# LauraBaracaldo/LauraBaracaldo-Spatial-Meta-Kriging-for-Distributed-Inference-for-Binary-Response

Measured on AMD Instinct MI355X. Metric: MCMC iters/sec (all subsets, whole node) + end-to-end wall-clock, n=500k K=250, higher is better.
Workload: dtype f64

## Files before the change

laurabaracaldo-spatial-meta-kriging-for-distributed-inference-for-binary-response_amd/csrc/mk_gemm.hpp:

```cpp
#pragma once
#include "mk_common.hpp"

namespace mk {

typedef double d4 __attribute__((ext_vector_type(4)));
typedef double d2 __attribute__((ext_vector_type(2)));

constexpr int GB_K = 16;
__host__ __device__ constexpr int gb_stride(int len) {
  return len == 256 ? 272 : (len == 128 ? 144 : (len == 64 ? 80 : 48));
}
__host__ __device__ constexpr int gb_img(int len) { return GB_K * gb_stride(len); }
__host__ __device__ constexpr int gb_lds_bytes(int tm, int tn) { return 2 * (gb_img(tm) + gb_img(tn)) * 8; }
static_assert(gb_lds_bytes(128, 128) == MK_GD_LDS_BYTES, "mk_common.hpp LDS size");
static_assert(128 * GB_K <= gb_img(128) && 64 * GB_K <= gb_img(64) && 32 * GB_K <= gb_img(32),
              "k-contiguous images fit their slots");

template <int BM, int BN>
struct AccT {
  d4 v[BM][BN];
};
typedef AccT<4, 4> Acc;

template <int BM, int BN>
__device__ inline void acc_zero(AccT<BM, BN>& a) {
#pragma unroll
  for (int i = 0; i < BM; ++i)
#pragma unroll
    for (int j = 0; j < BN; ++j) a.v[i][j] = (d4){0.0, 0.0, 0.0, 0.0};
}

__device__ inline int ku_swz(int m) { return (m >> 1) & 7; }

template <bool MU, int LEN>
__host__ __device__ constexpr int dma_count() { return MU ? 4 * (LEN > 128 ? LEN / 128 : 1) : (LEN + 31) / 32; }

template <bool MU, int LEN>
__device__ inline void dma_chunk(const double* __restrict__ X, long s, int k0, double* img) {
  const int w = threadIdx.x >> 6, lane = threadIdx.x & 63;
  if (MU) {
    static_assert(!MU || LEN <= 128 || LEN % 128 == 0, "m-contiguous rows of 128-double pieces");
#pragma unroll
    for (int j = 0; j < 4; ++j) {
      const int r = w + 4 * j;
#pragma unroll
      for (int pc = 0; pc < (LEN > 128 ? LEN / 128 : 1); ++pc)
        if (LEN >= 128 || lane < LEN / 2)
          __builtin_amdgcn_global_load_lds((const void*)(X + (long)(k0 + r) * s + 128 * pc + 2 * lane),
                                           (void*)(img + r * gb_stride(LEN) + 128 * pc), 16, 0, 0);
    }
  } else {
#pragma unroll
    for (int j = 0; j < (LEN + 31) / 32; ++j) {
// ... 116 lines not shown
  const int lane = threadIdx.x & 63, w = threadIdx.x >> 6;
  const int li = lane & 15, lk = lane >> 4;
#pragma unroll
  for (int ks = 0; ks < GB_K / 4; ++ks) {
    const int k = ks * 4 + lk;
    double ya[BM], xb[8];
#pragma unroll
    for (int b = 0; b < BM; ++b) {
      const double av = frag<true, TM>(As, w * (TM / 4) + b * 16 + li, k);
      ya[b] = NEG ? -av : av;
    }
#pragma unroll
    for (int b = 0; b < 8; ++b) xb[b] = frag<true, 128>(Bs, b * 16 + li, k);
#pragma unroll
    for (int bm = 0; bm < BM; ++bm)
#pragma unroll
      for (int bn = 0; bn < 8; ++bn)
        acc.v[bm][bn] = __builtin_amdgcn_mfma_f64_16x16x4f64(xb[bn], ya[bm], acc.v[bm][bn], 0, 0, 0);
  }
}

template <int TM, bool NEG>
__device__ inline void gemm_tile_rw(const double* __restrict__ A, long sA, const double* __restrict__ B, long sB, int K,
                                    AccRW<TM>& acc, double* lds) {
  constexpr int STAGE = gb_img(TM) + gb_img(128);
  const int nch = K / GB_K;
  auto issue = [&](int c) {
    double* st = lds + (c & 1) * STAGE;
    dma_chunk<true, TM>(A, sA, GB_K * c, st);
    dma_chunk<true, 128>(B, sB, GB_K * c, st + gb_img(TM));
  };
  issue(0);
  asm volatile("s_waitcnt vmcnt(0)" ::: "memory");
  __syncthreads();
  for (int c = 0; c < nch; ++c) {
    const double* st = lds + (c & 1) * STAGE;
    if (c + 1 < nch) issue(c + 1);
    mma_chunk_rw<TM, NEG>(st, st + gb_img(TM), acc);
    asm volatile("s_waitcnt vmcnt(0)" ::: "memory");
    __syncthreads();
  }
}

template <int TM>
__device__ inline void acc_load_rw(AccRW<TM>& acc, const double* C, long ldc) {
#pragma unroll
  for (int bm = 0; bm < TM / 64; ++bm)
#pragma unroll
    for (int bn = 0; bn < 8; ++bn)
#pragma unroll
      for (int r = 0; r < 4; ++r) acc.v[bm][bn][r] = C[rw_row<TM>(bm) + (long)rw_col(bn, r) * ldc];
}

template <bool A_MU, bool B_NU, bool NEG = false, bool REV = false, bool SAME = false, int SKIP = SKIP_NONE,
          bool MASK = false>
__device__ inline void gemm_128(const double* __restrict__ A, long sA, const double* __restrict__ B, long sB, int K,
                                int kvalid_total, Acc& acc, double* lds, int diag_tile = 0) {
  gemm_tile<128, 128, A_MU, B_NU, NEG, REV, SAME, SKIP, MASK>(A, sA, B, sB, K, kvalid_total, acc, lds, diag_tile);
}

template <int TM = 128>
__device__ inline int acc_row(int bm) {
  const int lane = threadIdx.x & 63, wm = (threadIdx.x >> 6) & 1;
  return wm * (TM / 2) + bm * 16 + (lane & 15);
}
template <int TN = 128>
__device__ inline int acc_col(int bn, int r) {
  const int lane = threadIdx.x & 63, wn = threadIdx.x >> 7;
  return wn * (TN / 2) + bn * 16 + (lane >> 4) + 4 * r;
}

template <int BM, int BN>
__device__ inline void acc_load(AccT<BM, BN>& acc, const double* C, long ldc) {
#pragma unroll
  for (int bm = 0; bm < BM; ++bm)
#pragma unroll
    for (int bn = 0; bn < BN; ++bn)
#pragma unroll
      for (int r = 0; r < 4; ++r) acc.v[bm][bn][r] = C[acc_row<BM * 32>(bm) + (long)acc_col<BN * 32>(bn, r) * ldc];
}

template <int BM, int BN>
__device__ inline void store_tile(double* C, long ldc, const AccT<BM, BN>& acc, double* Ct = nullptr) {
#pragma unroll
  for (int bm = 0; bm < BM; ++bm)
#pragma unroll
    for (int bn = 0; bn < BN; ++bn)
#pragma unroll
      for (int r = 0; r < 4; ++r) {
        const int m = acc_row<BM * 32>(bm), n = acc_col<BN * 32>(bn, r);
        C[m + (long)n * ldc] = acc.v[bm][bn][r];
        if (Ct) Ct[n + (long)m * ldc] = acc.v[bm][bn][r];
      }
}

constexpr int SYRK_SLOTS = 9;
__host__ __device__ constexpr int syrk_rb(int w, int s) { return s <= w ? w : 7 - w; }
__host__ __device__ constexpr int syrk_cb(int w, int s) { return s <= w ? s : s - w - 1; }
constexpr bool syrk_cover_exact() {
  int cnt[8][8] = {};
  for (int w = 0; w < 4; ++w)
    for (int s = 0; s < SYRK_SLOTS; ++s) {
      const int rb = syrk_rb(w, s), cb = syrk_cb(w, s);
      if (rb < 0 || rb > 7 || cb < 0 || cb > rb) return false;
      ++cnt[rb][cb];
    }
// ... 217 lines not shown
```

laurabaracaldo-spatial-meta-kriging-for-distributed-inference-for-binary-response_amd/csrc/mk_kernels.hpp:

```cpp
#pragma once
#include "mk_types.hpp"
#include "mk_corr.hpp"

namespace mk {
inline int xcd_grid_h(int S, int T) { return 8 * ((S + 7) / 8) * T; }
template <int MODEL>
__global__ void k_cov_candidate(Model md, MatSet ms, int h0, int hc, int which, int iter, const int* slist, const int* scount);
typedef void (*CovCandidateKernel)(Model, MatSet, int, int, int, int, const int*, const int*);
inline CovCandidateKernel cov_candidate_kernel(int model) {
  return model == MK_COV_EXPONENTIAL ? k_cov_candidate<MK_COV_EXPONENTIAL> : k_cov_candidate<MK_COV_MATERN>;
}
template <int TM, int TN = TM>
__global__ void k_chol_update(MatSet ms, int S, int h0, int hc, int k, int ia, int ib, int j0, int j1,
                              const int* slist, const int* scount, int syrk);
template <int TM>
__global__ void k_chol_trsm(MatSet ms, int S, int h0, int hc, int k, int ia, int ib, const int* slist,
                            const int* scount);
int pv_grid(int max_entries, int nt, int ntt);
template <int TM>
__global__ void k_chol_update_trsm(MatSet ms, int S, int h0, int hc, int k, int ia, int ib, int j0, int extra,
                                   const int* slist, const int* scount, int syrk);
__global__ void k_chol_diag(MatSet ms, const int* n_s, int h0, int hc, int k, double* ld_part, double* quad_c, int* info,
                            const int* slist, const int* scount, int cj0, int cj1, int syrk);
__global__ void k_inv_copydiag(MatSet ms, const int* list, const int* count);
template <int TM>
__global__ void k_inv_level(MatSet ms, const int* list, const int* count, int sz, int phase, int deal, int map);
__global__ void k_lauum(MatSet ms, const int* n_s, const int* list, const int* count);
__global__ void k_qblocks(MatSet ms, const int* n_s, const int* list, const int* count);
__global__ void k_take_border(Model md, MatSet ms, const int* list, const int* count, const double* zc);
__global__ void k_cand_border(Model md, MatSet ms, int h0, int hc);
__global__ void k_pred_draw_runs(Model md, const double* kz, const double* kA, int k_lo, const int* plist,
                                 const int* pcount, const int* run_start, int j_end);
__global__ void k_run_start(const int* plist, const int* pcount, int* run_start, int j);
__global__ void k_border_step(Model md, MatSet ms, int k);
__global__ void k_nu_border(Model md, MatSet ms);
__global__ void k_border_quad(Model md);
__global__ void k_trmv_Z(Model md, MatSet ms);
template <int MODEL>
__global__ void k_pred_PT(Model md, const int* list, const int* count);
__global__ void k_pred_PT_matern(Model md, const int* list, const int* count);
__global__ void k_matern_table(Model md, int h0, int hc, int which, int iter, const int* slist, const int* scount);
__global__ void k_matern_table_list(Model md, const int* list, const int* count);
typedef void (*PredPTKernel)(Model, const int*, const int*);
inline PredPTKernel pred_PT_kernel(int model) {
  return model == MK_COV_EXPONENTIAL ? k_pred_PT<MK_COV_EXPONENTIAL> : k_pred_PT<MK_COV_MATERN>;
}
template <bool GEN>
__global__ void k_pred_var(Model md, MatSet ms, const int* list, const int* count);
__global__ void k_pred_var_reduce(Model md, int nt, const int* list, const int* count);
__global__ void k_beta(Model md, int iter);
__global__ void k_Aphase(Model md, int iter);
__global__ void k_theta_mh(Model md, MatSet ms, int h0, int hc, int which, int iter);
__global__ void k_dirty_list(Model md, int force, int* list_inv, int* count_inv, int* list_pred, int* count_pred);
template <int Q>
__global__ void k_sweep(Model md, MatSet ms, int iter, const int* adm, int* fb);
template <int Q>
__global__ void k_sweep_mg(Model md, MatSet ms, int iter, double* part, int* cnt, int* xcc, int* err, int* adm, int spins_max);
template <int Q, int KR, int P, int HH, int LN>
__global__ void k_sweep_site(Model md, MatSet ms, int iter);
inline size_t sweep_site_lds_bytes(int ns_max, int q, int lean = 0) { return (size_t)ns_max * q * (lean ? 4 : 3) * 8 + (size_t)ns_max * 4; }
inline const void* sweep_site_kernel(int q, int kr, int lean = 1) {
  if (q == 1) {
    if (kr == 1)
      return lean == 1 ? (const void*)k_sweep_site<1, 4, 2, 0, 1> : (const void*)k_sweep_site<1, 4, 2, 0, 2>;
    return lean == 1 ? (const void*)k_sweep_site<1, 8, 2, 0, 1> : (const void*)k_sweep_site<1, 8, 2, 0, 2>;
  }
  switch (q) {
    case 2: return kr == 1 ? (const void*)k_sweep_site<2, 4, 1, 0, 0> : (const void*)k_sweep_site<2, 8, 1, 0, 0>;
    case 3: return kr == 1 ? (const void*)k_sweep_site<3, 4, 1, 0, 0> : nullptr;
    default: return nullptr;
  }
}
template <int Q>
__global__ void k_sweep_step(Model md, MatSet ms, int iter, int B, double* part);
// ... 72 lines not shown
```

laurabaracaldo-spatial-meta-kriging-for-distributed-inference-for-binary-response_amd/csrc/mk_linalg.hip:

```cpp
#include "mk_gemm.hpp"
#include "mk_types.hpp"
#include "mk_corr.hpp"

namespace mk {

__device__ inline void candidate_theta(const Model& md, int s, int h, int which, int iter, double* phi, double* nu) {
  const Key key = subset_key(md, s);
  const double* th = md.theta + (long)s * md.n_theta;
  const int idx_phi = md.ntri + h, idx_nu = md.ntri + md.q + h;
  double tphi = th[idx_phi];
  double tnu = (md.cov_model == MK_COV_MATERN) ? th[idx_nu] : 0.0;
  if (which == 0 || which == 1) {
    const int j_mh = (which == 0) ? md.o_phi + h : md.o_nu + h;
    const double z = proposal_normal(key, (uint32_t)j_mh, (uint32_t)iter);
    const double step = exp(md.tune[(long)s * md.n_mh_max + j_mh]) * z;
    if (which == 0) tphi += step; else tnu += step;
  }
  *phi = logit_inv(tphi, md.phi_a[h], md.phi_b[h]);
  *nu = (md.cov_model == MK_COV_MATERN) ? logit_inv(tnu, md.nu_a[h], md.nu_b[h]) : 0.0;
}

struct CandGen {
  const double* cx;
  const double* cy;
// ... 220 lines not shown
  const int sr = st % SUBR, sc = st / SUBR;
  const int i = ia + t;
  if (i == k && sc * TN >= (sr + 1) * TM) return;
  const int sh = s * ms.q + h;
  double* M = mat_slot(ms, sh, 1 - ms.cur[sh]);
  const long ld = ms.ld;
  double* C = M + i * MK_NB + sr * TM + (long)(k * MK_NB + sc * TN) * ld;
  const long jo = (long)j0 * MK_NB * ld;
  if (TM == 128 && TN == 128 && i == k && syrk) {
    AccSyrk a;
    acc_load_syrk(a, C, ld);
    gemm_syrk_128(M + i * MK_NB + jo, ld, (j1 - j0) * MK_NB, a, lds);
    store_tile_syrk(C, ld, a);
    return;
  }
  AccT<TM / 32, TN / 32> acc;
  acc_load(acc, C, ld);
  gemm_tile<TM, TN, true, true, true>(M + i * MK_NB + sr * TM + jo, ld, M + k * MK_NB + sc * TN + jo, ld,
                                      (j1 - j0) * MK_NB, (j1 - j0) * MK_NB, acc, lds);
  store_tile(C, ld, acc);
}
template __global__ void k_chol_update<128, 128>(MatSet, int, int, int, int, int, int, int, int, const int*, const int*, int);
template __global__ void k_chol_update<64, 64>(MatSet, int, int, int, int, int, int, int, int, const int*, const int*, int);
template __global__ void k_chol_update<32, 32>(MatSet, int, int, int, int, int, int, int, int, const int*, const int*, int);

template <int TM>
__global__ __launch_bounds__(256, 2) void k_chol_trsm(MatSet ms, int S, int h0, int hc, int k, int ia, int ib,
                                                     const int* slist, const int* scount) {
  extern __shared__ __attribute__((aligned(16))) double lds[];
  constexpr int SUB = MK_NB / TM;
  const int ntk = ib - ia;
  int e, t, s, h;
  if (!xcd_map(active_pairs(slist, scount, S, hc), ntk * SUB, &e, &t) || !pick_pair(slist, scount, e, h0, hc, &s, &h))
    return;
  const int sr = t % SUB;
  t /= SUB;
  const int i = ia + t;
  const int sh = s * ms.q + h;
  const int slot = 1 - ms.cur[sh];
  double* M = mat_slot(ms, sh, slot);
  const double* W = winv_slot(ms, sh, slot, k);
  const long ld = ms.ld;
  double* C = M + i * MK_NB + sr * TM + (long)k * MK_NB * ld;
  AccT<TM / 32, 4> acc;
  acc_zero(acc);
  gemm_tile<TM, 128, true, true, false, false, false, SKIP_TRI_B>(C, ld, W, MK_NB, MK_NB, MK_NB, acc, lds);
  store_tile(C, ld, acc);
}
template __global__ void k_chol_trsm<128>(MatSet, int, int, int, int, int, int, const int*, const int*);
template __global__ void k_chol_trsm<64>(MatSet, int, int, int, int, int, int, const int*, const int*);
template __global__ void k_chol_trsm<32>(MatSet, int, int, int, int, int, int, const int*, const int*);

template <int TM>
__global__ __launch_bounds__(256, 2) void k_chol_update_trsm(MatSet ms, int S, int h0, int hc, int k, int ia, int ib,
                                                            int j0, int extra, const int* slist, const int* scount,
                                                            int syrk) {
  extern __shared__ __attribute__((aligned(16))) double lds[];
  constexpr int SUB = MK_NB / TM, BM = TM / 64;
  const int ntk = ib - ia;
  int e, t, s, h;
  const int E = active_pairs(slist, scount, S, hc);
  if (!((extra && syrk) ? xcd_map_tail(E, ntk * SUB + extra, &e, &t) : xcd_map(E, ntk * SUB + extra, &e, &t)) ||
      !pick_pair(slist, scount, e, h0, hc, &s, &h))
    return;
  const int sh = s * ms.q + h;
  const int slot = 1 - ms.cur[sh];
  double* M = mat_slot(ms, sh, slot);
  const long ld = ms.ld;
  if (t == ntk * SUB) {
    double* C = M + ia * MK_NB + (long)ia * MK_NB * ld;
    if (syrk) {
      AccSyrk a;
      acc_load_syrk(a, C, ld);
      gemm_syrk_128(M + ia * MK_NB, ld, k * MK_NB, a, lds);
      store_tile_syrk(C, ld, a);
      return;
    }
    Acc acc;
    acc_load(acc, C, ld);
    gemm_tile<128, 128, true, true, true>(M + ia * MK_NB, ld, M + ia * MK_NB, ld, k * MK_NB, k * MK_NB, acc, lds);
    store_tile(C, ld, acc);
    return;
  }
  const int i = ia + t / SUB, r0 = i * MK_NB + (t % SUB) * TM;
  double* C = M + r0 + (long)k * MK_NB * ld;
  AccRW<TM> c;
  acc_load_rw<TM>(c, C, ld);
  const long jo = (long)j0 * MK_NB * ld;
  gemm_tile_rw<TM, true>(M + r0 + jo, ld, M + k * MK_NB + jo, ld, (k - j0) * MK_NB, c, lds);
  double* Co = C;
  long ldo = ld;
  asm volatile("" : "+s"(Co), "+s"(ldo));
  const double* Wt = winv_slot(ms, sh, slot, k);
  asm volatile("" : "+s"(Wt));
  constexpr int IMG = gb_img(32);
  auto issue = [&](int P, double* buf) {
#pragma nounroll
    for (int ch = 0; ch < 2 * P + 2; ++ch) dma_chunk<true, 32>(Wt + 32 * P, MK_NB, GB_K * ch, buf + ch * IMG);
  };
  double* bufA = lds;
  double* bufB = lds + 8 * IMG;
  issue(3, bufA);
  asm volatile("s_waitcnt vmcnt(0)" ::: "memory");
  __syncthreads();
  const int lane = threadIdx.x & 63, li = lane & 15, lk = lane >> 4;
#pragma unroll
  for (int idx = 0; idx < 4; ++idx) {
    const int P = idx == 0 ? 3 : (idx == 1 ? 0 : (idx == 2 ? 2 : 1));
    const double* buf = (idx & 1) ? bufB : bufA;
    if (idx < 3) {
      const int Pn = idx == 0 ? 0 : (idx == 1 ? 2 : 1);
      issue(Pn, (idx & 1) ? bufA : bufB);
    }
    AccT<BM, 2> o;
    acc_zero(o);
#pragma unroll
    for (int ch = 0; ch < 8; ++ch) {
      if (ch >= 2 * P + 2) break;
#pragma unroll
      for (int ks = 0; ks < GB_K / 4; ++ks) {
        const int kk = ks * 4 + lk;
        double xb[2];
#pragma unroll
        for (int b = 0; b < 2; ++b) xb[b] = frag<true, 32>(buf + ch * IMG, b * 16 + li, kk);
#pragma unroll
        for (int bm = 0; bm < BM; ++bm)
#pragma unroll
          for (int b = 0; b < 2; ++b) {
            if (ch > 2 * P + b) continue;
            o.v[bm][b] = __builtin_amdgcn_mfma_f64_16x16x4f64(xb[b], c.v[bm][ch][ks], o.v[bm][b], 0, 0, 0);
          }
      }
    }
#pragma unroll
    for (int bm = 0; bm < BM; ++bm)
#pragma unroll
      for (int b = 0; b < 2; ++b)
#pragma unroll
        for (int r = 0; r < 4; ++r) Co[rw_row<TM>(bm) + (long)rw_col(2 * P + b, r) * ldo] = o.v[bm][b][r];
    asm volatile("s_waitcnt vmcnt(0)" ::: "memory");
    __syncthreads();
  }
}
template __global__ void k_chol_update_trsm<128>(MatSet, int, int, int, int, int, int, int, int, const int*, const int*, int);
template __global__ void k_chol_update_trsm<64>(MatSet, int, int, int, int, int, int, int, int, const int*, const int*, int);

#define TLD MK_TLD
#define SLD 17
#ifdef MK_DIAG_TIMING
__device__ long long* mk_diag_ts;
#define MK_TSTAMP(i) do { if (threadIdx.x == 0) mk_diag_ts[blockIdx.x * 128 + (i)] = clock64(); } while (0)
#define MK_TSTAMPW(i, t) do { if (threadIdx.x == (t)) mk_diag_ts[blockIdx.x * 128 + (i)] = clock64(); } while (0)
#else
#define MK_TSTAMP(i) do { } while (0)
#define MK_TSTAMPW(i, t) do { } while (0)
#endif

__device__ inline double rlane(double v, int lane) {
  const long long b = __double_as_longlong(v);
  const int lo = __builtin_amdgcn_readlane((int)(b & 0xffffffffll), lane);
  const int hi = __builtin_amdgcn_readlane((int)(b >> 32), lane);
  return __longlong_as_double(((long long)hi << 32) | (unsigned)lo);
}

template <class FA, class FB>
__device__ inline d4 mfma16(d4 acc, int K, FA fa, FB fb) {
  const int l = threadIdx.x & 63;
  for (int k0 = 0; k0 < K; k0 += 16) {
    double a[4], b[4];
#pragma unroll
    for (int u = 0; u < 4; ++u) {
      a[u] = fa(l & 15, k0 + 4 * u + (l >> 4));
      b[u] = fb(k0 + 4 * u + (l >> 4), l & 15);
    }
#pragma unroll
    for (int u = 0; u < 4; ++u) acc = __builtin_amdgcn_mfma_f64_16x16x4f64(a[u], b[u], acc, 0, 0, 0);
  }
  return acc;
}

template <int N>
__device__ inline double bcast16_t(double v) { return __builtin_amdgcn_update_dpp(v, v, 0x150 + N, 0xf, 0xf, false); }
__device__ __forceinline__ double bcast16(double v, int n) {
  switch (n) {
    case 0: return bcast16_t<0>(v);   case 1: return bcast16_t<1>(v);   case 2: return bcast16_t<2>(v);
    case 3: return bcast16_t<3>(v);   case 4: return bcast16_t<4>(v);   case 5: return bcast16_t<5>(v);
    case 6: return bcast16_t<6>(v);   case 7: return bcast16_t<7>(v);   case 8: return bcast16_t<8>(v);
    case 9: return bcast16_t<9>(v);   case 10: return bcast16_t<10>(v); case 11: return bcast16_t<11>(v);
    case 12: return bcast16_t<12>(v); case 13: return bcast16_t<13>(v); case 14: return bcast16_t<14>(v);
    default: return bcast16_t<15>(v);
  }
}

__device__ inline void rsqrt_sqrt(double a, double* d, double* inv) {
  double y = __builtin_amdgcn_rsq(a);
  double e = fma(-a * y, y, 1.0);
  y = fma(0.5 * y, e, y);
  e = fma(-a * y, y, 1.0);
// ... 949 lines not shown
```

laurabaracaldo-spatial-meta-kriging-for-distributed-inference-for-binary-response_amd/csrc/mk_schedule.hip:

```cpp
#include <hip/hip_runtime.h>
#include <algorithm>
#include <cmath>
#include <vector>
#include "mk_gemm.hpp"
#include "mk_session.hpp"

using namespace mk;

void mk::drain_timers(mk_session* s) {
  std::vector<std::pair<float, float>> upd;
  for (auto& t : s->prof.pending) {
    hipEventSynchronize(t.b);
    float ms = 0.f;
    hipEventElapsedTime(&ms, t.a, t.b);
    if (t.cnt >= 0) t.flops *= (double)s->prof.inv_cnt[t.cnt];
    s->prof.stats[t.which].launches += 1;
    s->prof.stats[t.which].ms += ms;
    s->prof.stats[t.which].flops += t.flops;
    if (t.which == KS_CHOL_UPDATE || t.which == KS_CHOL_UPDATE_SUB) {
      float t0 = 0.f;
      hipEventElapsedTime(&t0, s->prof.pending.front().a, t.a);
      upd.push_back({t0, t0 + ms});
      s->prof.stats[KS_UPDATE_BUSY].launches += 1;
      s->prof.stats[KS_UPDATE_BUSY].flops += t.flops;
// ... 40 lines not shown
  return true;
}

int mk::launch_quantiles(unsigned grid, hipStream_t st, const double* data, long subset_stride, long row_stride,
                         int n_rows, int n_cols, const double* probs, int n_probs, double* out) {
  HIPCHK(hipFuncSetAttribute((const void*)k_quantiles, hipFuncAttributeMaxDynamicSharedMemorySize, MK_QUANT_MAX * 8));
  if (n_rows < 1 || n_rows > MK_QUANT_MAX)
    return set_err(MK_E_ARG, "quantile summaries take 1 .. " + std::to_string(MK_QUANT_MAX) + " kept samples");
  size_t n2 = 1;
  while (n2 < (size_t)n_rows) n2 <<= 1;
  MK_LAUNCH(k_quantiles, dim3(grid), dim3(256), n2 * 8, st, data, subset_stride, row_stride, n_rows, n_cols,
                     probs, n_probs, out);
  HIPCHK(hipGetLastError());
  return 0;
}

int mk::launch_quantiles_prob(unsigned grid, hipStream_t st, const double* data, long subset_stride, long row_stride,
                              int n_rows, int n_cols, const double* probs, int n_probs, double* out, const ProbSrc& ps) {
  HIPCHK(hipFuncSetAttribute((const void*)k_quantiles_prob, hipFuncAttributeMaxDynamicSharedMemorySize, MK_QUANT_MAX * 8));
  if (n_rows < 1 || n_rows > MK_QUANT_MAX)
    return set_err(MK_E_ARG, "quantile summaries take 1 .. " + std::to_string(MK_QUANT_MAX) + " kept samples");
  size_t n2 = 1;
  while (n2 < (size_t)n_rows) n2 <<= 1;
  MK_LAUNCH(k_quantiles_prob, dim3(grid), dim3(256), n2 * 8, st, data, subset_stride, row_stride, n_rows, n_cols,
                     probs, n_probs, out, ps);
  HIPCHK(hipGetLastError());
  return 0;
}

static int tile_size(long wg128) {
  static const int force = env_int("MK_TILE", 0);
  if (force == 32 || force == 64 || force == 128) return force;
  return wg128 >= 256 ? 128 : 64;
}

void mk::launch_candidates(const Model& md, const MatSet& ms, hipStream_t st, int n_entries, int h0, int hc, int which,
                           int iter, const int* slist, const int* scount) {
  if (md.cov_model == MK_COV_MATERN && md.chtab)
    MK_LAUNCH(k_matern_table, dim3(n_entries), dim3(256), 0, st, md, h0, hc, which, iter, slist, scount);
  const int ntiles = ms.nt * (ms.nt + 1) / 2;
  MK_LAUNCH(cov_candidate_kernel(md.cov_model), dim3(xcd_grid_h(n_entries, ntiles)),
                     dim3(256), 0, st, md, ms, h0, hc, which, iter, slist, scount);
}


static int diag_syrk() {
  static const int on = env_int("MK_DIAG_SYRK", 1);
  return on != 0;
}

static int inv_deal() {
  static const int on = env_int("MK_INV_DEAL", 1);
  return on != 0;
}

static int inv_map() {
  static const int on = env_int("MK_INV_MAP", 1);
  return on != 0;
}
static int inv_grid(int map, int max_entries, int nt, int sz, int sub) {
  if (map) return inv_map_grid(max_entries, nt, sz, sub);
  return xcd_grid_h(max_entries, (nt + 2 * sz - 1) / (2 * sz) * sz * sz * sub);
}
extern "C" int mk_inv_map_jobs(int32_t map, int32_t count, int32_t max_entries, int32_t nt, int32_t sz, int32_t phase,
                               int32_t sub, int32_t* out, int32_t cap) {
  const int grid = inv_grid(map, max_entries, nt, sz, sub);
  for (int b = 0; out && b < grid && b < cap; ++b) {
    int e, p, i, j, st;
    const bool job = map ? inv_map_job(count, nt, sz, phase, sub, b, &e, &p, &i, &j, &st)
                         : inv_xcd_job(count, nt, sz, phase, sub, b, &e, &p, &i, &j, &st);
    int32_t* o = out + 5 * (long)b;
    o[0] = job ? e : -1, o[1] = job ? p : -1, o[2] = job ? i : -1, o[3] = job ? j : -1, o[4] = job ? st : -1;
  }
  return grid;
}

static void chol_update(mk_session* s, Group& g, hipStream_t st, int h0, int hc, int k, int ia, int ib, int j0, int j1,
                        const int* slist, const int* scount, double flops) {
  const int E = g.S * hc, nti = ib - ia;
  if (nti <= 0) return;
  const int tm = tile_size((long)E * nti);
  if (tm == 32) {
    timed(s, st, KS_CHOL_UPDATE_SUB, flops, [&] {
      MK_LAUNCH(k_chol_update<32>, dim3(xcd_grid_h(E, nti * 16)), dim3(256), LDS_32, st, g.ms, g.S, h0, hc, k, ia,
                         ib, j0, j1, slist, scount, diag_syrk());
    });
  } else if (tm == 64) {
    timed(s, st, KS_CHOL_UPDATE_SUB, flops, [&] {
      MK_LAUNCH(k_chol_update<64>, dim3(xcd_grid_h(E, nti * 4)), dim3(256), LDS_64, st, g.ms, g.S, h0, hc, k, ia,
                         ib, j0, j1, slist, scount, diag_syrk());
    });
  } else {
    timed(s, st, KS_CHOL_UPDATE, flops, [&] {
      MK_LAUNCH(k_chol_update<128>, dim3(xcd_grid_h(E, nti)), dim3(256), LDS_128, st, g.ms, g.S, h0, hc, k, ia,
                         ib, j0, j1, slist, scount, diag_syrk());
    });
  }
}
static void chol_trsm(mk_session* s, Group& g, hipStream_t st, int h0, int hc, int k, int ia, int ib, const int* slist,
                      const int* scount, double flops) {
  const int E = g.S * hc, nti = ib - ia;
  if (nti <= 0) return;
  const int tm = tile_size((long)E * nti);
  timed(s, st, KS_CHOL_TRSM, flops, [&] {
    if (tm == 32)
      MK_LAUNCH(k_chol_trsm<32>, dim3(xcd_grid_h(E, nti * 4)), dim3(256), LDS_32x128, st, g.ms, g.S, h0, hc, k,
                         ia, ib, slist, scount);
    else if (tm == 64)
      MK_LAUNCH(k_chol_trsm<64>, dim3(xcd_grid_h(E, nti * 2)), dim3(256), LDS_64x128, st, g.ms, g.S, h0, hc, k,
                         ia, ib, slist, scount);
    else
      MK_LAUNCH(k_chol_trsm<128>, dim3(xcd_grid_h(E, nti)), dim3(256), LDS_128, st, g.ms, g.S, h0, hc, k, ia, ib,
                         slist, scount);
  });
}
static void chol_update_trsm(mk_session* s, Group& g, hipStream_t st, int h0, int hc, int k, int j0, int extra,
                             const int* slist, const int* scount, double flops) {
  const int E = g.S * hc, nt = s->nt, nti = nt - (k + 1);
  const int tm = tile_size((long)E * (nti + extra));
  timed(s, st, tm == 128 ? KS_CHOL_UPDATE : KS_CHOL_UPDATE_SUB, flops, [&] {
    if (tm == 128)
      MK_LAUNCH(k_chol_update_trsm<128>, dim3(xcd_grid_h(E, nti + extra)), dim3(256), LDS_128, st, g.ms, g.S, h0, hc,
                k, k + 1, nt, j0, extra, slist, scount, diag_syrk());
    else
      MK_LAUNCH(k_chol_update_trsm<64>, dim3(xcd_grid_h(E, 2 * nti + extra)), dim3(256), LDS_128, st, g.ms, g.S, h0,
                hc, k, k + 1, nt, j0, extra, slist, scount, diag_syrk());
  });
}
static void chol_diag(mk_session* s, Group& g, hipStream_t st, int h0, int hc, int k, const int* slist,
                      const int* scount, int cj0 = 0, int cj1 = 0, double flops = 0.0) {
  timed(s, st, KS_CHOL_DIAG, flops, [&] {
    MK_LAUNCH(k_chol_diag, dim3(g.S * hc), dim3(256), (size_t)MK_DIAG_LDS_BYTES, st, g.ms, g.md.n_s, h0, hc, k,
                       g.md.ld_part, g.md.quad_c, g.md.info, slist, scount, cj0, cj1, diag_syrk());
  });
}

static double panel_flops(mk_session* s, Group& g, int hc, int k, int ia, int ib, bool trsm, int j0 = 0, int j1 = -1) {
  if (j1 < 0) j1 = k;
  double fl = 0.0;
  for (int i = g.s0; i < g.s0 + g.S; ++i) {
    const double nv = (double)s->n_part[i] + 1.0;
    const double cols = std::fmin((double)MK_NB, std::fmax(0.0, nv - (double)k * MK_NB));
    const double depth = std::fmax(0.0, std::fmin((double)j1 * MK_NB, nv) - (double)j0 * MK_NB);
    const bool diag = ia <= k && k < ib;
    const double lo = (double)(diag ? k + 1 : ia) * MK_NB;
    const double rows = std::fmax(0.0, std::fmin(nv, (double)ib * MK_NB) - lo);
    if (trsm)
      fl += rows * cols * cols;
    else
      fl += 2.0 * rows * cols * depth + (diag ? cols * (cols + 1.0) * depth : 0.0);
  }
  return fl * hc;
}

static double inv_level_flops(int n, int nt, int sz, int phase) {
  double fl = 0.0;
  for (int T0 = 0; T0 < nt; T0 += 2 * sz) {
    const double t0 = (double)T0 * MK_NB, b0 = (double)(T0 + sz) * MK_NB, b1 = (double)(T0 + 2 * sz) * MK_NB;
    const double bt = std::fmax(0.0, std::fmin((double)n, b0) - t0), bb = std::fmax(0.0, std::fmin((double)n, b1) - b0);
    fl += phase == 0 ? bb * bt * bt : bb * bb * bt;
  }
  return fl;
}

void mk::launch_cholesky(mk_session* s, Group& g, int h0, int hc, const int* slist, const int* scount,
                         hipStream_t crit, hipEvent_t* evP, int k_lo, int k_hi) {
  const int nt = s->nt;
  if (k_hi < 0) k_hi = nt;
  hipStream_t A = crit ? crit : g.stream;
  static const int fused = env_int("MK_CHOL_FUSED", 1);
  if ((slist || !g.bulk) && fused) {
    for (int k = k_lo; k < k_hi; ++k) {
      const int j0 = k >= 2 ? k - 1 : 0;
      chol_diag(s, g, A, h0, hc, k, slist, scount, j0, k, k > 0 ? panel_flops(s, g, hc, k, k, k + 1, false, j0, k) : 0.0);
      if (k == 0 && nt > 1)
        chol_trsm(s, g, A, h0, hc, 0, 1, nt, slist, scount, panel_flops(s, g, hc, 0, 1, nt, true));
      else if (k > 0 && k < nt - 1)
        chol_update_trsm(s, g, A, h0, hc, k, 0, 1, slist, scount,
                         panel_flops(s, g, hc, k, k + 1, nt, false) + panel_flops(s, g, hc, k, k + 1, nt, true) +
// ... 370 lines not shown
```

laurabaracaldo-spatial-meta-kriging-for-distributed-inference-for-binary-response_amd/csrc/mk_types.hpp:

```cpp
#pragma once
#include "../../include/mk.h"
#include "mk_common.hpp"

#define MK_QMAX 4
#define MK_CD_SPLIT 8
#define MK_QUANT_MAX 16384

namespace mk {

struct Model {
  int S, q, p, n_pad, Np, nt, ntri, n_theta, cov_model;
  int link;
  int o_A, o_phi, o_nu, o_w, n_mh_max;
  int n_batch, batch_length, n_samples, kept0, n_kept;
  int n_test, n_test_pad, ntt;
  int subset_base;
  int S_all;
  int t_off;
  uint64_t seed;
  double accept_rate;
  double phi_a[MK_QMAX], phi_b[MK_QMAX], nu_a[MK_QMAX], nu_b[MK_QMAX];
  double iw_df, iw_S[MK_QMAX * MK_QMAX];
  const int* n_s;
  const double* coords;
// ... 77 lines not shown
  int p, link;
};

struct MapThr {
  double u[MK_MAP_MAXT];
  int J;
};

#define MK_CRIT_ACC 6
struct Crit {
  double* acc;
  double* part;
  double* sbeta;
  int nb;
  int n_cap;
};

__device__ inline long mat_elems(const MatSet& m) { return (long)m.ld * m.ld; }
__device__ inline double* mat_slot(const MatSet& m, int sh, int slot) {
  return m.L + ((long)sh * 2 + slot) * mat_elems(m);
}
__device__ inline double* winv_slot(const MatSet& m, int sh, int slot, int k) {
  return m.Winv + (((long)sh * 2 + slot) * m.nt + k) * (MK_NB * MK_NB);
}
__device__ inline Key subset_key(const Model& md, int s) { return make_key(md.seed, (uint32_t)(md.subset_base + s)); }

__host__ __device__ inline bool xcd_map_at(int b, int S, int T, int* s, int* t) {
  const int W = S * T, C = (W + 7) >> 3;
  const int x = b & 7, j = b >> 3;
  if (j >= C) return false;
  const int w = x * C + j;
  if (w >= W) return false;
  *s = w / T;
  *t = w % T;
  return true;
}
__device__ inline bool xcd_map(int S, int T, int* s, int* t) { return xcd_map_at(blockIdx.x, S, T, s, t); }
__device__ inline bool xcd_map_tail(int S, int T, int* s, int* t) {
  const int x = blockIdx.x & 7, j = blockIdx.x >> 3;
  const int Wr = S * (T - 1), Cr = (Wr + 7) >> 3, Cs = (S + 7) >> 3;
  if (j < Cr) {
    const int w = x * Cr + j;
    if (w >= Wr) return false;
    *s = w / (T - 1);
    *t = w % (T - 1);
    return true;
  }
  const int e = x * Cs + (j - Cr);
  if (j - Cr >= Cs || e >= S) return false;
  *s = e;
  *t = T - 1;
  return true;
}
__host__ inline int xcd_grid(int S, int T) { return 8 * ((S + 7) / 8) * T; }

struct InvShape {
  int sz, phase, sub, F, rl;
  __host__ __device__ int n(int k) const { return sub * (phase == 0 ? F * sz + rl : sz * (F + (rl >= k ? 1 : 0))); }
  __host__ __device__ int items() const { return sub * sz * (F * sz + rl); }
  __host__ __device__ int work() const {
    const int full = sz * (sz + 1) / 2;
    return sub * (phase == 0 ? (F * sz + rl) * full : sz * (F * full + rl * (rl + 1) / 2));
  }
};
__host__ __device__ inline InvShape inv_shape(int nt, int sz, int phase, int sub) {
  InvShape h;
  h.sz = sz;
  h.phase = phase;
  h.sub = sub;
  h.F = nt / (2 * sz);
  const int rem = nt - 2 * sz * h.F;
  h.rl = rem > sz ? rem - sz : 0;
  return h;
}
struct InvPos { int e, k, m; };
__host__ __device__ inline InvPos inv_map_cut(const InvShape& h, int S, int x) {
  InvPos q;
  q.e = (x * S) >> 3;
  const int tl = ((x * S) & 7) * h.work();
  int A = 0;
  for (int k = h.sz; k >= 1; --k) {
    const int nk = h.n(k), num = tl - 8 * A - 4 * k;
    if (nk > 0 && num <= 8 * k * (nk - 1)) {
      q.k = k;
      q.m = num <= 0 ? 0 : (num + 8 * k - 1) / (8 * k);
      return q;
    }
    A += nk * k;
  }
  q.e += 1;
  q.k = h.sz;
  q.m = 0;
  return q;
}
__host__ __device__ inline int inv_before(const InvShape& h, const InvPos& q, int k) {
  return k > q.k ? h.n(k) : (k == q.k ? q.m : 0);
}
__host__ __device__ inline bool inv_map_job(int S, int nt, int sz, int phase, int SUB, int b, int* e, int* p, int* i,
                                            int* j, int* st) {
  if (S <= 0) return false;
  const InvShape h = inv_shape(nt, sz, phase, SUB);
  const int x = b & 7;
  int q = b >> 3;
  const InvPos a = inv_map_cut(h, S, x), z = inv_map_cut(h, S, x + 1);
  for (int k = sz; k >= 1; --k) {
    const int nk = h.n(k), ba = inv_before(h, a, k);
// ... 47 lines not shown
```

Baseline: 12960.

## Skip padded rows in last Cholesky update-trsm tile for ragged subsets

For the 128-row update+trsm kernel, this computes how many 16-row blocks of the last row tile are real data for each subset (from n_s) and runs a column-split GEMM over only those blocks. Results are then reshuffled through LDS into the row-wise accumulator layout and passed to a shared solve epilogue that skips the dead row blocks. A new tail job map schedules the last two tiles separately. The intent is to stop spending MFMA work on padding rows in the ragged final tile, at the cost of an extra LDS transpose, more template instantiations and more register pressure.

```diff
diff --git a/laurabaracaldo-spatial-meta-kriging-for-distributed-inference-for-binary-response_amd/csrc/mk_gemm.hpp b/laurabaracaldo-spatial-meta-kriging-for-distributed-inference-for-binary-response_amd/csrc/mk_gemm.hpp
--- a/laurabaracaldo-spatial-meta-kriging-for-distributed-inference-for-binary-response_amd/csrc/mk_gemm.hpp
+++ b/laurabaracaldo-spatial-meta-kriging-for-distributed-inference-for-binary-response_amd/csrc/mk_gemm.hpp
@@ -1,4 +1,5 @@
 #pragma once
+#include <type_traits>
 #include "mk_common.hpp"
 
 namespace mk {
@@ -221,6 +222,99 @@
       for (int r = 0; r < 4; ++r) acc.v[bm][bn][r] = C[rw_row<TM>(bm) + (long)rw_col(bn, r) * ldc];
 }
 
+template <int V>
+using AccCS = AccT<V, 2>;
+constexpr int CS_VMAX = 6;
+
+template <int V, bool NEG>
+__device__ inline void mma_chunk_cs(const double* As, const double* Bs, AccCS<V>& acc, int w) {
+  const int lane = threadIdx.x & 63;
+  const int li = lane & 15, lk = lane >> 4;
+#pragma unroll
+  for (int ks = 0; ks < GB_K / 4; ++ks) {
+    const int k = ks * 4 + lk;
+    double ya[V], xb[2];
+#pragma unroll
+    for (int b = 0; b < V; ++b) {
+      const double av = frag<true, 128>(As, b * 16 + li, k);
+      ya[b] = NEG ? -av : av;
+    }
+#pragma unroll
+    for (int j = 0; j < 2; ++j) xb[j] = frag<true, 128>(Bs, (2 * w + j) * 16 + li, k);
+#pragma unroll
+    for (int bm = 0; bm < V; ++bm)
+#pragma unroll
+      for (int j = 0; j < 2; ++j)
+        acc.v[bm][j] = __builtin_amdgcn_mfma_f64_16x16x4f64(xb[j], ya[bm], acc.v[bm][j], 0, 0, 0);
+  }
+}
+
+template <int V, bool NEG>
+__device__ inline void gemm_tile_cs(const double* __restrict__ A, long sA, const double* __restrict__ B, long sB, int K,
+                                    AccCS<V>& acc, double* lds, int w) {
+  constexpr int STAGE = 2 * gb_img(128);
+  const int nch = K / GB_K;
+  auto issue = [&](int c) {
+    double* st = lds + (c & 1) * STAGE;
+    dma_chunk<true, 128>(A, sA, GB_K * c, st);
+    dma_chunk<true, 128>(B, sB, GB_K * c, st + gb_img(128));
+  };
+  issue(0);
+  asm volatile("s_waitcnt vmcnt(0)" ::: "memory");
+  __syncthreads();
+  for (int c = 0; c < nch; ++c) {
+    const double* st = lds + (c & 1) * STAGE;
+    if (c + 1 < nch) issue(c + 1);
+    mma_chunk_cs<V, NEG>(st, st + gb_img(128), acc, w);
+    asm volatile("s_waitcnt vmcnt(0)" ::: "memory");
+    __syncthreads();
+  }
+}
+
+template <int V>
+__device__ inline void acc_load_cs(AccCS<V>& acc, const double* C, long ldc, int w) {
+  const int li = threadIdx.x & 15, lk = (threadIdx.x & 63) >> 4;
+#pragma unroll
+  for (int bm = 0; bm < V; ++bm)
+#pragma unroll
+    for (int j = 0; j < 2; ++j)
+#pragma unroll
+      for (int r = 0; r < 4; ++r) acc.v[bm][j][r] = C[16 * bm + li + (long)(16 * (2 * w + j) + lk + 4 * r) * ldc];
+}
+
+template <int V>
+__device__ inline void cs_to_rw(const AccCS<V>& a, AccRW<128>& c, double* lds, int w) {
+  static_assert(V >= 1 && V <= 7 && 4 * V * 2048 <= gb_lds_bytes(128, 128), "a round fits the stages' LDS");
+  d2* img = (d2*)lds;
+  const int lane = threadIdx.x & 63;
+#pragma unroll
+  for (int j = 0; j < 2; ++j) {
+#pragma unroll
+    for (int bm = 0; bm < V; ++bm) {
+      d2* p = img + ((bm * 4 + w) * 64 + lane) * 2;
+      p[0] = (d2){a.v[bm][j][0], a.v[bm][j][1]};
+      p[1] = (d2){a.v[bm][j][2], a.v[bm][j][3]};
+    }
+    __syncthreads();
+#pragma unroll
+    for (int bm = 0; bm < 2; ++bm) {
+      const int rb = 2 * w + bm;
+      if (rb < V) {
+#pragma unroll
+        for (int ws = 0; ws < 4; ++ws) {
+          const d2* p = img + ((rb * 4 + ws) * 64 + lane) * 2;
+          const d2 lo = p[0], hi = p[1];
+          c.v[bm][2 * ws + j] = (d4){lo[0], lo[1], hi[0], hi[1]};
+        }
+      } else {
+#pragma unroll
+        for (int ws = 0; ws < 4; ++ws) c.v[bm][2 * ws + j] = (d4){0.0, 0.0, 0.0, 0.0};
+      }
+    }
+    __syncthreads();
+  }
+}
+
 template <bool A_MU, bool B_NU, bool NEG = false, bool REV = false, bool SAME = false, int SKIP = SKIP_NONE,
           bool MASK = false>
 __device__ inline void gemm_128(const double* __restrict__ A, long sA, const double* __restrict__ B, long sB, int K,
diff --git a/laurabaracaldo-spatial-meta-kriging-for-distributed-inference-for-binary-response_amd/csrc/mk_kernels.hpp b/laurabaracaldo-spatial-meta-kriging-for-distributed-inference-for-binary-response_amd/csrc/mk_kernels.hpp
--- a/laurabaracaldo-spatial-meta-kriging-for-distributed-inference-for-binary-response_amd/csrc/mk_kernels.hpp
+++ b/laurabaracaldo-spatial-meta-kriging-for-distributed-inference-for-binary-response_amd/csrc/mk_kernels.hpp
@@ -19,7 +19,7 @@
 int pv_grid(int max_entries, int nt, int ntt);
 template <int TM>
 __global__ void k_chol_update_trsm(MatSet ms, int S, int h0, int hc, int k, int ia, int ib, int j0, int extra,
-                                   const int* slist, const int* scount, int syrk);
+                                   const int* slist, const int* scount, int syrk, const int* n_s, int ragged);
 __global__ void k_chol_diag(MatSet ms, const int* n_s, int h0, int hc, int k, double* ld_part, double* quad_c, int* info,
                             const int* slist, const int* scount, int cj0, int cj1, int syrk);
 __global__ void k_inv_copydiag(MatSet ms, const int* list, const int* count);
diff --git a/laurabaracaldo-spatial-meta-kriging-for-distributed-inference-for-binary-response_amd/csrc/mk_linalg.hip b/laurabaracaldo-spatial-meta-kriging-for-distributed-inference-for-binary-response_amd/csrc/mk_linalg.hip
--- a/laurabaracaldo-spatial-meta-kriging-for-distributed-inference-for-binary-response_amd/csrc/mk_linalg.hip
+++ b/laurabaracaldo-spatial-meta-kriging-for-distributed-inference-for-binary-response_amd/csrc/mk_linalg.hip
@@ -296,17 +296,81 @@
 template __global__ void k_chol_trsm<32>(MatSet, int, int, int, int, int, int, const int*, const int*);
 
 template <int TM>
+__device__ inline void solve_epilogue_rw(const AccRW<TM>& c, int nbm, double* C, long ld, const double* Wt, double* lds) {
+  constexpr int BM = TM / 64;
+  double* Co = C;
+  long ldo = ld;
+  asm volatile("" : "+s"(Co), "+s"(ldo));
+  asm volatile("" : "+s"(Wt));
+  constexpr int IMG = gb_img(32);
+  auto issue = [&](int P, double* buf) {
+#pragma nounroll
+    for (int ch = 0; ch < 2 * P + 2; ++ch) dma_chunk<true, 32>(Wt + 32 * P, MK_NB, GB_K * ch, buf + ch * IMG);
+  };
+  double* bufA = lds;
+  double* bufB = lds + 8 * IMG;
+  issue(3, bufA);
+  asm volatile("s_waitcnt vmcnt(0)" ::: "memory");
+  __syncthreads();
+  const int lane = threadIdx.x & 63, li = lane & 15, lk = lane >> 4;
+#pragma unroll
+  for (int idx = 0; idx < 4; ++idx) {
+    const int P = idx == 0 ? 3 : (idx == 1 ? 0 : (idx == 2 ? 2 : 1));
+    const double* buf = (idx & 1) ? bufB : bufA;
+    if (idx < 3) {
+      const int Pn = idx == 0 ? 0 : (idx == 1 ? 2 : 1);
+      issue(Pn, (idx & 1) ? bufA : bufB);
+    }
+    AccT<BM, 2> o;
+    acc_zero(o);
+#pragma unroll
+    for (int ch = 0; ch < 8; ++ch) {
+      if (ch >= 2 * P + 2 || nbm == 0) break;
+#pragma unroll
+      for (int ks = 0; ks < GB_K / 4; ++ks) {
+        const int kk = ks * 4 + lk;
+        double xb[2];
+#pragma unroll
+        for (int b = 0; b < 2; ++b) xb[b] = frag<true, 32>(buf + ch * IMG, b * 16 + li, kk);
+#pragma unroll
+        for (int bm = 0; bm < BM; ++bm)
+#pragma unroll
+          for (int b = 0; b < 2; ++b) {
+            if (ch > 2 * P + b) continue;
+            o.v[bm][b] = __builtin_amdgcn_mfma_f64_16x16x4f64(xb[b], c.v[bm][ch][ks], o.v[bm][b], 0, 0, 0);
+          }
+      }
+    }
+#pragma unroll
+    for (int bm = 0; bm < BM; ++bm) {
+      if (bm >= nbm) break;
+#pragma unroll
+      for (int b = 0; b < 2; ++b)
+#pragma unroll
+        for (int r = 0; r < 4; ++r) Co[rw_row<TM>(bm) + (long)rw_col(2 * P + b, r) * ldo] = o.v[bm][b][r];
+    }
+    asm volatile("s_waitcnt vmcnt(0)" ::: "memory");
+    __syncthreads();
+  }
+}
+
+template <int TM>
 __global__ __launch_bounds__(256, 2) void k_chol_update_trsm(MatSet ms, int S, int h0, int hc, int k, int ia, int ib,
                                                             int j0, int extra, const int* slist, const int* scount,
-                                                            int syrk) {
+                                                            int syrk, const int* __restrict__ n_s, int ragged) {
   extern __shared__ __attribute__((aligned(16))) double lds[];
   constexpr int SUB = MK_NB / TM, BM = TM / 64;
   const int ntk = ib - ia;
   int e, t, s, h;
   const int E = active_pairs(slist, scount, S, hc);
-  if (!((extra && syrk) ? xcd_map_tail(E, ntk * SUB + extra, &e, &t) : xcd_map(E, ntk * SUB + extra, &e, &t)) ||
-      !pick_pair(slist, scount, e, h0, hc, &s, &h))
-    return;
+  bool job;
+  if (TM == 128 && extra && syrk && ragged == 2 && ntk >= 2)
+    job = xcd_map_tail2(E, ntk + extra, &e, &t);
+  else if (extra && syrk)
+    job = xcd_map_tail(E, ntk * SUB + extra, &e, &t);
+  else
+    job = xcd_map(E, ntk * SUB + extra, &e, &t);
+  if (!job || !pick_pair(slist, scount, e, h0, hc, &s, &h)) return;
   const int sh = s * ms.q + h;
   const int slot = 1 - ms.cur[sh];
   double* M = mat_slot(ms, sh, slot);
@@ -328,66 +392,43 @@
   }
   const int i = ia + t / SUB, r0 = i * MK_NB + (t % SUB) * TM;
   double* C = M + r0 + (long)k * MK_NB * ld;
+  const long jo = (long)j0 * MK_NB * ld;
+  const double* Wt = winv_slot(ms, sh, slot, k);
+  if constexpr (TM == 128) {
+    const int v = ragged ? (n_s[s] + 1 - i * MK_NB + 15) >> 4 : 8;
+    if (v >= 1 && v <= CS_VMAX) {
+      const int w = syrk_wave();
+      auto run = [&](auto vt) {
+        constexpr int V = decltype(vt)::value;
+        AccRW<128> c;
+        {
+          AccCS<V> a;
+          acc_load_cs<V>(a, C, ld, w);
+          gemm_tile_cs<V, true>(M + r0 + jo, ld, M + k * MK_NB + jo, ld, (k - j0) * MK_NB, a, lds, w);
+          cs_to_rw<V>(a, c, lds, w);
+        }
+        solve_epilogue_rw<128>(c, min(max(V - 2 * w, 0), 2), C, ld, Wt, lds);
+      };
+      switch (v) {
+        case 1: run(std::integral_constant<int, 1>{}); break;
+        case 2: run(std::integral_constant<int, 2>{}); break;
+        case 3: run(std::integral_constant<int, 3>{}); break;
+        case 4: run(std::integral_constant<int, 4>{}); break;
+        case 5: run(std::integral_constant<int, 5>{}); break;
+        default: run(std::integral_constant<int, 6>{}); break;
+      }
+      return;
+    }
+  }
   AccRW<TM> c;
   acc_load_rw<TM>(c, C, ld);
-  const long jo = (long)j0 * MK_NB * ld;
   gemm_tile_rw<TM, true>(M + r0 + jo, ld, M + k * MK_NB + jo, ld, (k - j0) * MK_NB, c, lds);
-  double* Co = C;
-  long ldo = ld;
-  asm volatile("" : "+s"(Co), "+s"(ldo));
-  const double* Wt = winv_slot(ms, sh, slot, k);
-  asm volatile("" : "+s"(Wt));
-  constexpr int IMG = gb_img(32);
-  auto issue = [&](int P, double* buf) {
-#pragma nounroll
-    for (int ch = 0; ch < 2 * P + 2; ++ch) dma_chunk<true, 32>(Wt + 32 * P, MK_NB, GB_K * ch, buf + ch * IMG);
-  };
-  double* bufA = lds;
-  double* bufB = lds + 8 * IMG;
-  issue(3, bufA);
-  asm volatile("s_waitcnt vmcnt(0)" ::: "memory");
-  __syncthreads();
-  const int lane = threadIdx.x & 63, li = lane & 15, lk = lane >> 4;
-#pragma unroll
-  for (int idx = 0; idx < 4; ++idx) {
-    const int P = idx == 0 ? 3 : (idx == 1 ? 0 : (idx == 2 ? 2 : 1));
-    const double* buf = (idx & 1) ? bufB : bufA;
-    if (idx < 3) {
-      const int Pn = idx == 0 ? 0 : (idx == 1 ? 2 : 1);
-      issue(Pn, (idx & 1) ? bufA : bufB);
-    }
-    AccT<BM, 2> o;
-    acc_zero(o);
-#pragma unroll
-    for (int ch = 0; ch < 8; ++ch) {
-      if (ch >= 2 * P + 2) break;
-#pragma unroll
-      for (int ks = 0; ks < GB_K / 4; ++ks) {
-        const int kk = ks * 4 + lk;
-        double xb[2];
-#pragma unroll
-        for (int b = 0; b < 2; ++b) xb[b] = frag<true, 32>(buf + ch * IMG, b * 16 + li, kk);
-#pragma unroll
-        for (int bm = 0; bm < BM; ++bm)
-#pragma unroll
-          for (int b = 0; b < 2; ++b) {
-            if (ch > 2 * P + b) continue;
-            o.v[bm][b] = __builtin_amdgcn_mfma_f64_16x16x4f64(xb[b], c.v[bm][ch][ks], o.v[bm][b], 0, 0, 0);
-          }
-      }
-    }
-#pragma unroll
-    for (int bm = 0; bm < BM; ++bm)
-#pragma unroll
-      for (int b = 0; b < 2; ++b)
-#pragma unroll
-        for (int r = 0; r < 4; ++r) Co[rw_row<TM>(bm) + (long)rw_col(2 * P + b, r) * ldo] = o.v[bm][b][r];
-    asm volatile("s_waitcnt vmcnt(0)" ::: "memory");
-    __syncthreads();
-  }
-}
-template __global__ void k_chol_update_trsm<128>(MatSet, int, int, int, int, int, int, int, int, const int*, const int*, int);
-template __global__ void k_chol_update_trsm<64>(MatSet, int, int, int, int, int, int, int, int, const int*, const int*, int);
+  solve_epilogue_rw<TM>(c, BM, C, ld, Wt, lds);
+}
+template __global__ void k_chol_update_trsm<128>(MatSet, int, int, int, int, int, int, int, int, const int*, const int*, int,
+                                                 const int*, int);
+template __global__ void k_chol_update_trsm<64>(MatSet, int, int, int, int, int, int, int, int, const int*, const int*, int,
+                                                const int*, int);
 
 #define TLD MK_TLD
 #define SLD 17
diff --git a/laurabaracaldo-spatial-meta-kriging-for-distributed-inference-for-binary-response_amd/csrc/mk_schedule.hip b/laurabaracaldo-spatial-meta-kriging-for-distributed-inference-for-binary-response_amd/csrc/mk_schedule.hip
--- a/laurabaracaldo-spatial-meta-kriging-for-distributed-inference-for-binary-response_amd/csrc/mk_schedule.hip
+++ b/laurabaracaldo-spatial-meta-kriging-for-distributed-inference-for-binary-response_amd/csrc/mk_schedule.hip
@@ -116,6 +116,18 @@
 static int inv_deal() {
   static const int on = env_int("MK_INV_DEAL", 1);
   return on != 0;
+}
+
+static int ragged() {
+  static const int on = env_int("MK_RAGGED", 1);
+  return on != 0;
+}
+static int ragged_arg(mk_session* s, const Group& g) {
+  if (!ragged()) return 0;
+  int nmax = 0;
+  for (int i = g.s0; i < g.s0 + g.S; ++i) nmax = std::max(nmax, (int)s->n_part[i]);
+  const int v = (nmax + 1 - (s->nt - 1) * MK_NB + 15) / 16;
+  return v >= 1 && v <= CS_VMAX ? 2 : 1;
 }
 
 static int inv_map() {
@@ -185,10 +197,10 @@
   timed(s, st, tm == 128 ? KS_CHOL_UPDATE : KS_CHOL_UPDATE_SUB, flops, [&] {
     if (tm == 128)
       MK_LAUNCH(k_chol_update_trsm<128>, dim3(xcd_grid_h(E, nti + extra)), dim3(256), LDS_128, st, g.ms, g.S, h0, hc,
-                k, k + 1, nt, j0, extra, slist, scount, diag_syrk());
+                k, k + 1, nt, j0, extra, slist, scount, diag_syrk(), g.md.n_s, ragged_arg(s, g));
     else
       MK_LAUNCH(k_chol_update_trsm<64>, dim3(xcd_grid_h(E, 2 * nti + extra)), dim3(256), LDS_128, st, g.ms, g.S, h0,
-                hc, k, k + 1, nt, j0, extra, slist, scount, diag_syrk());
+                hc, k, k + 1, nt, j0, extra, slist, scount, diag_syrk(), g.md.n_s, 0);
   });
 }
 static void chol_diag(mk_session* s, Group& g, hipStream_t st, int h0, int hc, int k, const int* slist,
diff --git a/laurabaracaldo-spatial-meta-kriging-for-distributed-inference-for-binary-response_amd/csrc/mk_types.hpp b/laurabaracaldo-spatial-meta-kriging-for-distributed-inference-for-binary-response_amd/csrc/mk_types.hpp
--- a/laurabaracaldo-spatial-meta-kriging-for-distributed-inference-for-binary-response_amd/csrc/mk_types.hpp
+++ b/laurabaracaldo-spatial-meta-kriging-for-distributed-inference-for-binary-response_amd/csrc/mk_types.hpp
@@ -153,6 +153,26 @@
   *t = T - 1;
   return true;
 }
+__device__ inline bool xcd_map_tail2(int S, int T, int* s, int* t) {
+  const int x = blockIdx.x & 7;
+  int j = blockIdx.x >> 3;
+  const int Wr = S * (T - 2), Cr = (Wr + 7) >> 3, Cs = (S + 7) >> 3;
+  if (j < Cr) {
+    const int w = x * Cr + j;
+    if (w >= Wr) return false;
+    *s = w / (T - 2);
+    *t = w % (T - 2);
+    return true;
+  }
+  j -= Cr;
+  if (j >= 2 * Cs) return false;
+  const int cls = j >= Cs ? 1 : 0;
+  const int e = x * Cs + (j - cls * Cs);
+  if (e >= S) return false;
+  *s = e;
+  *t = T - 2 + cls;
+  return true;
+}
 __host__ inline int xcd_grid(int S, int T) { return 8 * ((S + 7) / 8) * T; }
 
 struct InvShape {
```

New measurement: 13250, median of 6. 1.02x the previous value.
